# index-tts/index-tts

Measured on AMD Instinct MI355X. Metric: audio-seconds/sec (RTF) IndexTTS-2.5, 64-utt batch @1/2/4/8 MI355X, higher is better.
Workload: dtype bf16 (GPT GEMM operands / KV cache; f32 accumulate, residual stream, norms: the reference's own GPU mode) + fp32x3 (flow matching: f32 activations / weights / accumulation, GEMM and attention products on the bf16 matrix pipe with every f32 operand carried exactly as three bf16 planes = 24 significan

## Files before the change

### indextts_amd/csrc/bigvgan_kernels.hip

```cpp
#include "bigvgan_kernels.h"
#include <stdlib.h>

#define AA_TILE 1024

__global__ __launch_bounds__(256) void aa_act_kernel(const float* __restrict__ x, float* __restrict__ y,
                                                     const float* __restrict__ alpha, const float* __restrict__ beta,
                                                     const float* __restrict__ fu, const float* __restrict__ fd,
                                                     int C, int T, const int* __restrict__ lens, int len_mult,
                                                     int logscale) {
    __shared__ float xs[AA_TILE + 16];
    __shared__ float vs[2 * AA_TILE + 16];
    __shared__ float fus[12], fds[12];
    const int b = blockIdx.z, c = blockIdx.y;
    const int t0 = blockIdx.x * AA_TILE;
    const int len = lens ? min(lens[b] * len_mult, T) : T;
    if (t0 >= len) return;
    const int tid = threadIdx.x;
    if (tid < 12) { fus[tid] = fu[tid]; fds[tid] = fd[tid]; }
    const float* xr = x + ((size_t)b * C + c) * T;
    float* yr = y + ((size_t)b * C + c) * T;
    float a_e = alpha[c], b_e = beta[c];
    if (logscale) { a_e = expf(a_e); b_e = expf(b_e); }
    const float inv_b = 1.0f / (b_e + 1e-9f);
    const int n_out = min(AA_TILE, len - t0);
    for (int i = tid; i < n_out + 12; i += 256) {
        int t = t0 - 6 + i;
        t = t < 0 ? 0 : (t > len - 1 ? len - 1 : t);
        xs[i] = xr[t];
    }
    __syncthreads();
    const int two_len_m1 = 2 * len - 1;
    for (int vi = tid; vi < 2 * n_out + 12; vi += 256) {
        int i = 2 * t0 - 6 + vi;
        i = i < 0 ? 0 : (i > two_len_m1 ? two_len_m1 : i);
        const int q = i >> 1;
        const int base = q - (t0 - 6);
        float u = 0.f;
        if (i & 1) {
#pragma unroll
            for (int j = 0; j < 6; ++j) u = fmaf(fus[2 * j], xs[base + 3 - j], u);
        } else {
#pragma unroll
            for (int j = 0; j < 6; ++j) u = fmaf(fus[1 + 2 * j], xs[base + 2 - j], u);
        }
        u *= 2.0f;
        const float s = sinf(u * a_e);
        vs[vi] = u + inv_b * s * s;
    }
    __syncthreads();
    for (int i = tid; i < n_out; i += 256) {
        float acc = 0.f;
#pragma unroll
        for (int j = 0; j < 12; ++j) acc = fmaf(fds[j], vs[2 * i + j + 1], acc);
        yr[t0 + i] = acc;
    }
}

__device__ __forceinline__ float sin_reduced(float x) {
    const float inv2pi = 0.15915494309189535f;
    const float k = rintf(x * inv2pi);
    float r = fmaf(-k, 6.2831855f, x);
    r = fmaf(-k, -1.7484555e-7f, r);
    return __builtin_amdgcn_sinf(r * inv2pi);
}

__device__ __forceinline__ int aa_sw(int i) { return i ^ (((i >> 6) & 1) << 2); }

template <int OPT, bool FAST_SIN>
__global__ __launch_bounds__(256) void aa_act_kernel_v2(const float* __restrict__ x, float* __restrict__ y,
                                                        const float* __restrict__ alpha, const float* __restrict__ beta,
                                                        const float* __restrict__ fu, const float* __restrict__ fd,
                                                        int C, int T, const int* __restrict__ lens, int len_mult,
                                                        int logscale) {
    constexpr int TILE = 256 * OPT;
    __shared__ __attribute__((aligned(16))) float xs[TILE + 16];
    __shared__ __attribute__((aligned(16))) float vs[2 * TILE + 64];
    const int b = blockIdx.z, c = blockIdx.y;
    const int t0 = blockIdx.x * TILE;
    const int len = lens ? min(lens[b] * len_mult, T) : T;
    if (t0 >= len) return;
    const int tid = threadIdx.x;
    const float* xr = x + ((size_t)b * C + c) * T;
    float* yr = y + ((size_t)b * C + c) * T;
    float fus[12], fds[12];
#pragma unroll
    for (int j = 0; j < 12; ++j) { fus[j] = 2.0f * fu[j]; fds[j] = fd[j]; }
    float a_e = alpha[c], b_e = beta[c];
    if (logscale) { a_e = expf(a_e); b_e = expf(b_e); }
    const float inv_b = 1.0f / (b_e + 1e-9f);
    const int n_out = min(TILE, len - t0);
    float xl[OPT + 1];
#pragma unroll
    for (int k = 0; k < OPT + 1; ++k) {
        int t = t0 - 6 + tid + 256 * k;
        t = t < 0 ? 0 : (t > len - 1 ? len - 1 : t);
        xl[k] = xr[t];
    }
#pragma unroll
    for (int k = 0; k < OPT + 1; ++k)
        if (tid + 256 * k < TILE + 12) xs[tid + 256 * k] = xl[k];
    __syncthreads();
    auto snake8 = [&](int vb, float* v) {
        float xw[12];
        *(f32x4*)&xw[0] = *(const f32x4*)&xs[(vb >> 1)];
        *(f32x4*)&xw[4] = *(const f32x4*)&xs[(vb >> 1) + 4];
        *(f32x4*)&xw[8] = *(const f32x4*)&xs[(vb >> 1) + 8];
#pragma unroll
        for (int p = 0; p < 4; ++p) {
            float ue = 0.f, uo = 0.f;
#pragma unroll
            for (int j = 0; j < 6; ++j) {
                ue = fmaf(fus[1 + 2 * j], xw[p + 5 - j], ue);
                uo = fmaf(fus[2 * j], xw[p + 6 - j], uo);
            }
            const float se = FAST_SIN ? sin_reduced(ue * a_e) : sinf(ue * a_e);
            const float so = FAST_SIN ? sin_reduced(uo * a_e) : sinf(uo * a_e);
            v[2 * p] = fmaf(inv_b * se, se, ue);
            v[2 * p + 1] = fmaf(inv_b * so, so, uo);
        }
    };
#pragma unroll
    for (int g = 0; g < OPT / 4; ++g) {
        float v[8];
        const int vb = 2 * OPT * tid + 8 * g;
        snake8(vb, v);
        *(f32x4*)&vs[aa_sw(vb)] = *(const f32x4*)&v[0];
        *(f32x4*)&vs[aa_sw(vb + 4)] = *(const f32x4*)&v[4];
    }
    if (tid < 2) {
        float vt[8];
        snake8(2 * TILE + 8 * tid, vt);
        *(f32x4*)&vs[aa_sw(2 * TILE + 8 * tid)] = *(const f32x4*)&vt[0];
        *(f32x4*)&vs[aa_sw(2 * TILE + 8 * tid + 4)] = *(const f32x4*)&vt[4];
    }
    __syncthreads();
    if (t0 == 0 && tid < 6) vs[aa_sw(tid)] = vs[aa_sw(6)];
    const int vi_end = (2 * len - 1) - (2 * t0 - 6);
    if (vi_end < 2 * TILE + 12 - 1) {
        const int vi = vi_end + 1 + tid;
        if (tid < 8 && vi < 2 * TILE + 16) vs[aa_sw(vi)] = vs[aa_sw(vi_end)];
    }
    __syncthreads();
#pragma unroll
    for (int g = 0; g < OPT / 4; ++g) {
        float vw[20];
        const int base = 2 * (OPT * tid + 4 * g);
#pragma unroll
        for (int k = 0; k < 5; ++k) *(f32x4*)&vw[4 * k] = *(const f32x4*)&vs[aa_sw(base + 4 * k)];
        f32x4 o;
#pragma unroll
        for (int p = 0; p < 4; ++p) {
            float acc = 0.f;
#pragma unroll
            for (int j = 0; j < 12; ++j) acc = fmaf(fds[j], vw[2 * p + j + 1], acc);
            o[p] = acc;
        }
        const int i0 = OPT * tid + 4 * g;
        if (i0 + 3 < n_out && ((t0 + i0) & 3) == 0 && (T & 3) == 0) {
            *(f32x4*)&yr[t0 + i0] = o;
        } else {
#pragma unroll
            for (int p = 0; p < 4; ++p)
                if (i0 + p < n_out) yr[t0 + i0 + p] = o[p];
        }
    }
}

#define AAP_TT 128
#define AAP_CB 32
#define AAP_RS 36
__device__ __forceinline__ uint32_t aap_cvt2(float a, float b) {
    typedef __bf16 bf2 __attribute__((ext_vector_type(2)));
    typedef float f2 __attribute__((ext_vector_type(2)));
    return __builtin_bit_cast(uint32_t, __builtin_convertvector(f2{a, b}, bf2));
}
__device__ __forceinline__ void aap_wave_sync() {
    __builtin_amdgcn_fence(__ATOMIC_RELEASE, "wavefront");
    __builtin_amdgcn_wave_barrier();
    __builtin_amdgcn_fence(__ATOMIC_ACQUIRE, "wavefront");
}
__device__ __forceinline__ int aap_slot(int tt) { return (tt & 3) * 32 + (tt >> 2); }

__global__ __launch_bounds__(256) void aa_act_planes_kernel(const float* __restrict__ x, u16* __restrict__ xh, u16* __restrict__ xm, u16* __restrict__ xl,
                                                            const float* __restrict__ alpha, const float* __restrict__ beta,
                                                            const float* __restrict__ fu, const float* __restrict__ fd,
                                                            int C, int T, const int* __restrict__ lens, int len_mult, int logscale) {
    __shared__ __attribute__((aligned(256))) float xs[4][2][192];
    __shared__ __attribute__((aligned(256))) float vs[4][2][320];
    __shared__ __attribute__((aligned(16))) u16 ot[3][AAP_TT][AAP_RS];
    const int b = blockIdx.z, c0 = blockIdx.y * AAP_CB, t0 = blockIdx.x * AAP_TT;
    const int tid = threadIdx.x, lane = tid & 63, w = tid >> 6, sub = lane >> 5, pos = lane & 31;
    const int len = lens ? min(lens[b] * len_mult, T) : T;
    const int n_out = len - t0 < AAP_TT ? (len - t0 < 0 ? 0 : len - t0) : AAP_TT;
    if (n_out > 0) {
        float fus[12], fds[12];
#pragma unroll
        for (int j = 0; j < 12; ++j) { fus[j] = 2.0f * fu[j]; fds[j] = fd[j]; }
        float* xw_ = xs[w][sub];
        float* vw_ = vs[w][sub];
        int toff[5];
#pragma unroll
        for (int k = 0; k < 5; ++k) {
            int t = t0 - 6 + pos + 32 * k;
            toff[k] = t < 0 ? 0 : (t > len - 1 ? len - 1 : t);
        }
        auto chan = [&](int it) { const int c = c0 + w * 8 + it * 2 + sub; return c < C ? c : C - 1; };
        float xn[5];
        {
            const float* xr = x + ((size_t)b * C + chan(0)) * T;
#pragma unroll
            for (int k = 0; k < 5; ++k) xn[k] = xr[toff[k]];
        }
#pragma unroll 1
        for (int it = 0; it < 4; ++it) {
            const int cl = w * 8 + it * 2 + sub;
            const bool c_ok = c0 + cl < C;
            float a_e = alpha[chan(it)], b_e = beta[chan(it)];
            if (logscale) { a_e = expf(a_e); b_e = expf(b_e); }
            const float inv_b = 1.0f / (b_e + 1e-9f);
            aap_wave_sync();
#pragma unroll
            for (int k = 0; k < 5; ++k) xw_[pos + 32 * k] = xn[k];
            if (it < 3) {
                const float* xr = x + ((size_t)b * C + chan(it + 1)) * T;
#pragma unroll
                for (int k = 0; k < 5; ++k) xn[k] = xr[toff[k]];
            }
            aap_wave_sync();
            auto snake8 = [&](int vb, float* v) {
                float xw[12];
                *(f32x4*)&xw[0] = *(const f32x4*)&xw_[(vb >> 1)];
                *(f32x4*)&xw[4] = *(const f32x4*)&xw_[(vb >> 1) + 4];
                *(f32x4*)&xw[8] = *(const f32x4*)&xw_[(vb >> 1) + 8];
#pragma unroll
                for (int p = 0; p < 4; ++p) {
                    float ue = 0.f, uo = 0.f;
#pragma unroll
                    for (int j = 0; j < 6; ++j) {
                        ue = fmaf(fus[1 + 2 * j], xw[p + 5 - j], ue);
                        uo = fmaf(fus[2 * j], xw[p + 6 - j], uo);
                    }
                    const float se = sin_reduced(ue * a_e);
                    const float so = sin_reduced(uo * a_e);
                    v[2 * p] = fmaf(inv_b * se, se, ue);
                    v[2 * p + 1] = fmaf(inv_b * so, so, uo);
                }
            };
            {
                float v[8];
                const int vb = 8 * pos;
                snake8(vb, v);
                *(f32x4*)&vw_[aa_sw(vb)] = *(const f32x4*)&v[0];
                *(f32x4*)&vw_[aa_sw(vb + 4)] = *(const f32x4*)&v[4];
            }
            if (pos < 2) {
                float vt[8];
                snake8(2 * AAP_TT + 8 * pos, vt);
                *(f32x4*)&vw_[aa_sw(2 * AAP_TT + 8 * pos)] = *(const f32x4*)&vt[0];
                *(f32x4*)&vw_[aa_sw(2 * AAP_TT + 8 * pos + 4)] = *(const f32x4*)&vt[4];
            }
            aap_wave_sync();
            if (t0 == 0 && pos < 6) vw_[aa_sw(pos)] = vw_[aa_sw(6)];
            const int vi_end = (2 * len - 1) - (2 * t0 - 6);
            if (vi_end < 2 * AAP_TT + 12 - 1) {
                const int vi = vi_end + 1 + pos;
                if (pos < 8 && vi < 2 * AAP_TT + 16) vw_[aa_sw(vi)] = vw_[aa_sw(vi_end)];
            }
            aap_wave_sync();
            float vw[20];
            const int base = 8 * pos;
#pragma unroll
            for (int k = 0; k < 5; ++k) *(f32x4*)&vw[4 * k] = *(const f32x4*)&vw_[aa_sw(base + 4 * k)];
            float o[4];
#pragma unroll
            for (int p = 0; p < 4; ++p) {
                float acc = 0.f;
#pragma unroll
                for (int j = 0; j < 12; ++j) acc = fmaf(fds[j], vw[2 * p + j + 1], acc);
                o[p] = (4 * pos + p < n_out && c_ok) ? acc : 0.f;
            }
#pragma unroll
            for (int e = 0; e < 2; ++e) {
                const float f0 = o[2 * e], f1 = o[2 * e + 1];
                const uint32_t h = aap_cvt2(f0, f1);
                const float r0 = f0 - __uint_as_float(h << 16), r1 = f1 - __uint_as_float(h & 0xffff0000u);
                const uint32_t m = aap_cvt2(r0, r1);
                const float s0 = r0 - __uint_as_float(m << 16), s1 = r1 - __uint_as_float(m & 0xffff0000u);
                const uint32_t l = aap_cvt2(s0, s1);
                const int sa = aap_slot(4 * pos + 2 * e), sb = aap_slot(4 * pos + 2 * e + 1);
                ot[0][sa][cl] = (u16)h; ot[0][sb][cl] = (u16)(h >> 16);
                ot[1][sa][cl] = (u16)m; ot[1][sb][cl] = (u16)(m >> 16);
                ot[2][sa][cl] = (u16)l; ot[2][sb][cl] = (u16)(l >> 16);
            }
        }
    }
    __syncthreads();
    const size_t plane_row = (size_t)b * T;
    const int q = tid & 3;
#pragma unroll 1
    for (int r = tid >> 2; r < 3 * AAP_TT; r += 64) {
        const int p = r / AAP_TT, tt = r - p * AAP_TT;
        const int t = t0 + tt;
        if (t >= T || c0 + 8 * q >= C) continue;
        uint2 lo = {0u, 0u}, hi = {0u, 0u};
        if (n_out > 0) {
            const u16* src = &ot[p][aap_slot(tt)][8 * q];
            lo = *(const uint2*)src;
            hi = *(const uint2*)(src + 4);
        }
        u16* dst = (p == 0 ? xh : (p == 1 ? xm : xl)) + (plane_row + t) * C + c0 + 8 * q;
        *(uint4*)dst = uint4{lo.x, lo.y, hi.x, hi.y};
    }
}

#define CI_CHUNK 32
#define CONV_HALO 64


template <int WM, int WN, int MT, int NT>
__global__ __launch_bounds__(256) __attribute__((amdgpu_waves_per_eu((WM == 1 && MT == 1) ? 4 : 1, (WM == 1 && MT == 1) ? 4 : 8)))
void conv_mfma_kernel(ConvArgs a) {
    constexpr int BM = WM * MT * 32;
    constexpr int BN = WN * NT * 32;
    constexpr int LDW = BN + CONV_HALO;
    extern __shared__ __attribute__((aligned(16))) float xs[];

    const int tid = threadIdx.x, lane = tid & 63, w = tid >> 6;
    const int wm = w / WN, wn = w % WN;
    const int L = blockIdx.x;
    const int xcd = L & 7, slot = L >> 3;
    const int tile = (slot / a.n_co) * 8 + xcd;
    if (tile >= a.n_mt * a.B) return;
    const int b = tile / a.n_mt;
    const int m0 = (tile - b * a.n_mt) * BN;
    const int co0 = (slot % a.n_co) * BM;
    const int len_in = a.lens ? min(a.lens[b] * a.len_mult_in, a.Tin) : a.Tin;
    const int len_out = a.lens ? min(a.lens[b] * a.len_mult_out, a.Tout) : a.Tout;
    const int m_count = len_in + a.m_extra;
    if (m0 >= m_count) return;

    const int span = (a.k - 1) * (a.tap_step < 0 ? -a.tap_step : a.tap_step);
    const int last_off = a.tap_base + (a.k - 1) * a.tap_step;
    const int min_off = a.tap_base < last_off ? a.tap_base : last_off;
    const int W = BN + span;
    const int n_cosub = (a.Cout + 31) >> 5;
    const int cin8 = a.Cin >> 3;

    f32x16 acc[MT][NT];
#pragma unroll
    for (int i = 0; i < MT; ++i)
#pragma unroll
        for (int j = 0; j < NT; ++j)
#pragma unroll
            for (int r = 0; r < 16; ++r) acc[i][j][r] = 0.f;

    const float* xb = a.x + (size_t)b * a.Cin * a.Tin;
    const int lane_row = lane >> 5;
    const int lane_col = lane & 31;

    constexpr int NCOL = LDW / 64;
    float stage[CI_CHUNK / 4][NCOL];
    const int w_u = __builtin_amdgcn_readfirstlane(w);
    auto stage_load = [&](int ci0s) {
        const int cnt = min(CI_CHUNK, a.Cin - ci0s);
#pragma unroll
        for (int rr = 0; rr < CI_CHUNK / 4; ++rr) {
            const int r = w_u + 4 * rr;
            const bool row_ok = r < cnt;
            const float* xr = xb + (size_t)(ci0s + (row_ok ? r : 0)) * a.Tin;
            const __amdgpu_buffer_rsrc_t rsrc =
                __builtin_amdgcn_make_buffer_rsrc(const_cast<float*>(xr), 0, row_ok ? len_in * 4 : 0, 0x00020000);
#pragma unroll
            for (int i = 0; i < NCOL; ++i) {
                const int t = m0 + min_off + lane + 64 * i;
                stage[rr][i] = __builtin_bit_cast(float, __builtin_amdgcn_raw_buffer_load_b32(rsrc, t * 4, 0, 0));
            }
        }
    };
    auto stage_write = [&]() {
#pragma unroll
        for (int rr = 0; rr < CI_CHUNK / 4; ++rr)
#pragma unroll
            for (int i = 0; i < NCOL; ++i) xs[(w + 4 * rr) * LDW + lane + 64 * i] = stage[rr][i];
    };
    stage_load(0);

    constexpr int CP4 = CI_CHUNK / 8;
    f32x4 a_cur[CP4][MT], a_nxt[CP4][MT];
    const int nchunks = (a.Cin + CI_CHUNK - 1) / CI_CHUNK;
    const int G = nchunks * a.k;
    const unsigned wpk_bytes = (unsigned)n_cosub * a.k * cin8 * 64u * 16u;
    const __amdgpu_buffer_rsrc_t wrs = __builtin_amdgcn_make_buffer_rsrc(const_cast<float*>(a.wpk), 0, (int)wpk_bytes, 0x00020000);
    auto load_tap = [&](int g, f32x4 (&dst)[CP4][MT]) {
        const int c = g / a.k, j = g - c * a.k;
        const int cbase = c * CI_CHUNK;
        const int cp4n = min(CI_CHUNK, a.Cin - cbase) >> 3;
#pragma unroll
        for (int cp4 = 0; cp4 < CP4; ++cp4) {
#pragma unroll
            for (int mt = 0; mt < MT; ++mt) {
                const int co_sub = (co0 >> 5) + wm * MT + mt;
                const bool ok = (cp4 < cp4n) && (co_sub < n_cosub);
                const unsigned off = ok ? ((unsigned)((co_sub * a.k + j) * cin8 + ((cbase >> 3) + cp4)) * 64u + lane) * 16u
                                        : 0xFFFFFFF0u;
                dst[cp4][mt] = __builtin_bit_cast(f32x4, __builtin_amdgcn_raw_buffer_load_b128(wrs, off, 0, 0));
            }
        }
    };
    auto compute_tap = [&](int j) {
        const int colb = wn * NT * 32 + lane_col + (a.tap_base + j * a.tap_step - min_off);
        const float* xcol = xs + lane_row * LDW + colb;
        float bcur[4][NT], bnxt[4][NT];
#pragma unroll
        for (int sidx = 0; sidx < 4; ++sidx)
#pragma unroll
            for (int nt = 0; nt < NT; ++nt) bcur[sidx][nt] = xcol[(2 * sidx) * LDW + nt * 32];
#pragma unroll
        for (int cp4 = 0; cp4 < CP4; ++cp4) {
            if (cp4 + 1 < CP4) {
#pragma unroll
                for (int sidx = 0; sidx < 4; ++sidx)
#pragma unroll
                    for (int nt = 0; nt < NT; ++nt) bnxt[sidx][nt] = xcol[((cp4 + 1) * 8 + 2 * sidx) * LDW + nt * 32];
            }
#pragma unroll
            for (int sidx = 0; sidx < 4; ++sidx)
#pragma unroll
                for (int mt = 0; mt < MT; ++mt)
#pragma unroll
                    for (int nt = 0; nt < NT; ++nt)
                        acc[mt][nt] = __builtin_amdgcn_mfma_f32_32x32x2f32(a_cur[cp4][mt][sidx], bcur[sidx][nt], acc[mt][nt], 0, 0, 0);
            if (cp4 + 1 < CP4) {
#pragma unroll
                for (int sidx = 0; sidx < 4; ++sidx)
#pragma unroll
                    for (int nt = 0; nt < NT; ++nt) bcur[sidx][nt] = bnxt[sidx][nt];
            }
        }
#pragma unroll
        for (int cp4 = 0; cp4 < CP4; ++cp4)
#pragma unroll
            for (int mt = 0; mt < MT; ++mt) a_cur[cp4][mt] = a_nxt[cp4][mt];
    };
    load_tap(0, a_cur);
    int g = 0;
    for (int ci0 = 0; ci0 < a.Cin; ci0 += CI_CHUNK) {
        __syncthreads();
        stage_write();
        __syncthreads();
        load_tap(g + 1 < G ? g + 1 : G - 1, a_nxt);
        stage_load(ci0 + CI_CHUNK);
        compute_tap(0);
        ++g;
        for (int j = 1; j < a.k; ++j, ++g) {
            load_tap(g + 1 < G ? g + 1 : G - 1, a_nxt);
            compute_tap(j);
        }
    }

    const int plane_bytes = a.Cout * a.Tout * 4;
    const __amdgpu_buffer_rsrc_t yrs =
        __builtin_amdgcn_make_buffer_rsrc(a.y + (size_t)b * a.Cout * a.Tout, 0, plane_bytes, 0x00020000);
    const float* resb = a.res ? a.res + (size_t)b * a.Cout * a.Tout : a.y;
    const __amdgpu_buffer_rsrc_t rrs = __builtin_amdgcn_make_buffer_rsrc(const_cast<float*>(resb), 0, plane_bytes, 0x00020000);
#pragma unroll
    for (int mt = 0; mt < MT; ++mt) {
#pragma unroll
        for (int hf = 0; hf < 2; ++hf) {
            int corow[8];
            float badd[8];
#pragma unroll
            for (int q = 0; q < 8; ++q) {
                const int r = hf * 8 + q;
                corow[q] = co0 + (wm * MT + mt) * 32 + (r & 3) + 8 * (r >> 2) + 4 * lane_row;
                badd[q] = 0.f;
            }
            if (a.bias) {
#pragma unroll
                for (int q = 0; q < 8; ++q) badd[q] = a.bias[corow[q] < a.Cout ? corow[q] : a.Cout - 1];
            }
            if (a.bias_b) {
                const float* bb = a.bias_b + (size_t)b * a.Cout;
#pragma unroll
                for (int q = 0; q < 8; ++q) badd[q] += bb[corow[q] < a.Cout ? corow[q] : a.Cout - 1];
            }
#pragma unroll
            for (int nt = 0; nt < NT; ++nt) {
                const int m = m0 + (wn * NT + nt) * 32 + lane_col;
                const int n = m * a.ostride + a.ooff;
                const bool n_ok = (m < m_count) && (n >= 0) && (n < len_out);
                unsigned voff[8];
                float v[8];
#pragma unroll
                for (int q = 0; q < 8; ++q) {
                    const bool ok = n_ok && corow[q] < a.Cout;
                    voff[q] = ok ? (unsigned)(corow[q] * a.Tout + n) * 4u : 0xFFFFFFF0u;
                    v[q] = acc[mt][nt][hf * 8 + q] + badd[q];
                }
                if (a.res) {
                    float rv[8];
#pragma unroll
                    for (int q = 0; q < 8; ++q) rv[q] = __builtin_bit_cast(float, __builtin_amdgcn_raw_buffer_load_b32(rrs, voff[q], 0, 0));
#pragma unroll
                    for (int q = 0; q < 8; ++q) v[q] += rv[q];
                }
                if (a.acc_mode != 0) {
                    float yo[8];
#pragma unroll
                    for (int q = 0; q < 8; ++q) yo[q] = __builtin_bit_cast(float, __builtin_amdgcn_raw_buffer_load_b32(yrs, voff[q], 0, 0));
#pragma unroll
                    for (int q = 0; q < 8; ++q) v[q] = a.acc_mode == 1 ? yo[q] + v[q] : (yo[q] + v[q]) / a.div;
                }
#pragma unroll
                for (int q = 0; q < 8; ++q) __builtin_amdgcn_raw_buffer_store_b32(__builtin_bit_cast(unsigned, v[q]), yrs, voff[q], 0, 0);
            }
        }
    }
}

__global__ __launch_bounds__(256) void conv_post_kernel(const float* __restrict__ x, float* __restrict__ y,
                                                        const float* __restrict__ w, const float* __restrict__ bias,
                                                        int Cin, int T, int k, const int* __restrict__ lens,
                                                        int len_mult, int use_tanh) {
    extern __shared__ float ws[];
    const int b = blockIdx.y;
    for (int i = threadIdx.x; i < Cin * k; i += 256) ws[i] = w[i];
    __syncthreads();
    const int t = blockIdx.x * 256 + threadIdx.x;
    if (t >= T) return;
    const int len = lens ? min(lens[b] * len_mult, T) : T;
    float acc = 0.f;
    if (t < len) {
        const int pad = (k - 1) / 2;
        acc = bias ? bias[0] : 0.f;
        const float* xb = x + (size_t)b * Cin * T;
        for (int ci = 0; ci < Cin; ++ci) {
            const float* xr = xb + (size_t)ci * T;
            for (int j = 0; j < k; ++j) {
                const int tt = t + j - pad;
                if (tt >= 0 && tt < len) acc = fmaf(ws[ci * k + j], xr[tt], acc);
            }
        }
        acc = use_tanh ? tanhf(acc) : fminf(1.0f, fmaxf(-1.0f, acc));
    }
    y[(size_t)b * T + t] = acc;
}

__global__ __launch_bounds__(256) void cond_bias_kernel(const float* __restrict__ spk, const float* __restrict__ w,
                                                        const float* __restrict__ bias, float* __restrict__ out,
                                                        int Cout, int cond_dim) {
    const int b = blockIdx.y;
    const int co = blockIdx.x * 256 + threadIdx.x;
    if (co >= Cout) return;
    float acc = bias ? bias[co] : 0.f;
    const float* wr = w + (size_t)co * cond_dim;
    const float* sr = spk + (size_t)b * cond_dim;
    for (int d = 0; d < cond_dim; ++d) acc = fmaf(wr[d], sr[d], acc);
    out[(size_t)b * Cout + co] = acc;
}

int launch_aa_act(const float* x, float* y, const float* alpha, const float* beta, const float* fu, const float* fd,
                  int B, int C, int T, const int* lens, int len_mult, int logscale, hipStream_t st) {
    if (B <= 0 || C <= 0 || T <= 0) return ITTS_OK;
    const int mode = itts_opt(OPT_AA_ACT);
    if (mode == 0) hipLaunchKernelGGL(aa_act_kernel, dim3(ceil_div(T, AA_TILE), C, B), dim3(256), 0, st, x, y, alpha, beta, fu, fd, C, T, lens, len_mult, logscale);
    else if (mode == 1) hipLaunchKernelGGL((aa_act_kernel_v2<4, false>), dim3(ceil_div(T, 1024), C, B), dim3(256), 0, st, x, y, alpha, beta, fu, fd, C, T, lens, len_mult, logscale);
    else if (mode == 2) hipLaunchKernelGGL((aa_act_kernel_v2<4, true>), dim3(ceil_div(T, 1024), C, B), dim3(256), 0, st, x, y, alpha, beta, fu, fd, C, T, lens, len_mult, logscale);
    else hipLaunchKernelGGL((aa_act_kernel_v2<8, true>), dim3(ceil_div(T, 2048), C, B), dim3(256), 0, st, x, y, alpha, beta, fu, fd, C, T, lens, len_mult, logscale);
    HIP_TRY(hipGetLastError());
    return ITTS_OK;
}

int launch_aa_act_planes(const float* x, void* xp, const float* alpha, const float* beta, const float* fu, const float* fd,
                         int B, int C, int T, const int* lens, int len_mult, int logscale, hipStream_t st) {
    if (B <= 0 || C <= 0 || T <= 0) return ITTS_OK;
    if (C % 8) { itts_set_error("aa_act_planes: C %% 8 != 0"); return ITTS_ERR_ARG; }
    u16* p = (u16*)xp;
    const size_t plane = (size_t)B * T * C;
    hipLaunchKernelGGL(aa_act_planes_kernel, dim3(ceil_div(T, AAP_TT), ceil_div(C, AAP_CB), B), dim3(256), 0, st, x, p, p + plane, p + 2 * plane,
                       alpha, beta, fu, fd, C, T, lens, len_mult, logscale);
    HIP_TRY(hipGetLastError());
    return ITTS_OK;
}

template <int WM, int WN, int MT, int NT>
static int launch_conv_cfg(const ConvArgs& a, int B, int m_total, hipStream_t st) {
    constexpr int BM = WM * MT * 32, BN = WN * NT * 32;
    const size_t lds = (size_t)CI_CHUNK * (BN + CONV_HALO) * sizeof(float);
    ConvArgs a2 = a;
    a2.B = B;
    a2.n_mt = ceil_div(m_total, BN);
    a2.n_co = ceil_div(a.Cout, BM);
    const long long tiles8 = ((long long)a2.n_mt * B + 7) / 8 * 8;
    const long long nblocks = tiles8 * a2.n_co;
    if (nblocks > 2147483647ll) { itts_set_error("conv: grid too large"); return ITTS_ERR_ARG; }
    hipLaunchKernelGGL((conv_mfma_kernel<WM, WN, MT, NT>), dim3((unsigned)nblocks), dim3(256), lds, st, a2);
    HIP_TRY(hipGetLastError());
    return ITTS_OK;
}

int launch_conv(const ConvArgs& a, int B, hipStream_t st) {
    if (B <= 0) return ITTS_OK;
    if (a.Cin % 8 != 0) { itts_set_error("conv: C_in=%d must be a multiple of 8", a.Cin); return ITTS_ERR_ARG; }
    if ((long long)a.Cout * a.Tout >= (1ll << 29)) { itts_set_error("conv: C_out*T_out = %lld exceeds the 2 GiB per-row plane limit", (long long)a.Cout * a.Tout); return ITTS_ERR_ARG; }
    if ((long long)a.Tin >= (1ll << 29)) { itts_set_error("conv: T too large"); return ITTS_ERR_ARG; }
    const int span = (a.k - 1) * (a.tap_step < 0 ? -a.tap_step : a.tap_step);
    if (span > CONV_HALO) { itts_set_error("conv: tap span %d exceeds halo %d", span, CONV_HALO); return ITTS_ERR_ARG; }
    const int m_total = a.Tin + a.m_extra;
    const int n_cosub = (a.Cout + 31) / 32;
    const int force_bm = itts_opt(OPT_CONV_BM);
    const int bm_sub = force_bm ? force_bm / 32 : 1;
    (void)n_cosub;
    switch (bm_sub) {
        case 1: return launch_conv_cfg<1, 4, 1, 2>(a, B, m_total, st);
        case 2: return launch_conv_cfg<1, 4, 2, 2>(a, B, m_total, st);
        case 3: return launch_conv_cfg<1, 4, 3, 2>(a, B, m_total, st);
        default: return launch_conv_cfg<2, 2, 2, 2>(a, B, m_total, st);
    }
}

int launch_conv_post(const float* x, float* y, const float* w, const float* bias, int B, int Cin, int T, int k,
                     const int* lens, int len_mult, int use_tanh, hipStream_t st) {
    if (B <= 0 || T <= 0) return ITTS_OK;
    dim3 grid(ceil_div(T, 256), B);
    hipLaunchKernelGGL(conv_post_kernel, grid, dim3(256), (size_t)Cin * k * sizeof(float), st, x, y, w, bias, Cin, T, k,
                       lens, len_mult, use_tanh);
    HIP_TRY(hipGetLastError());
    return ITTS_OK;
}

int launch_cond_bias(const float* spk, const float* w, const float* bias, float* out, int B, int Cout, int cond_dim,
                     hipStream_t st) {
    if (B <= 0 || Cout <= 0) return ITTS_OK;
    dim3 grid(ceil_div(Cout, 256), B);
    hipLaunchKernelGGL(cond_bias_kernel, grid, dim3(256), 0, st, spk, w, bias, out, Cout, cond_dim);
    HIP_TRY(hipGetLastError());
    return ITTS_OK;
}
```

### indextts_amd/csrc/common.h

```cpp
#pragma once
#include <hip/hip_runtime.h>
#include <stdint.h>
#include <stdio.h>
#include <string.h>

#define ITTS_OK 0
#define ITTS_ERR_ARG 1
#define ITTS_ERR_HIP 2
#define ITTS_ERR_STATE 3
#define ITTS_ERR_NOMEM 4

#define HIP_TRY(expr)                                                                         \
    do {                                                                                      \
        hipError_t _e = (expr);                                                               \
        if (_e != hipSuccess) {                                                               \
            itts_set_error("%s:%d %s -> %s", __FILE__, __LINE__, #expr, hipGetErrorString(_e)); \
            return ITTS_ERR_HIP;                                                              \
        }                                                                                     \
    } while (0)

void itts_set_error(const char* fmt, ...);

enum { OPT_DECODE_FUSE_LN, OPT_DECODE_GEMM, OPT_DECODE_ROT, OPT_DECODE_WNT, OPT_DECODE_NT, OPT_PREFILL_GEMM, OPT_TILE256, OPT_F32_TILE,
       OPT_X3_PRODUCTS, OPT_X3_SCHED, OPT_X3_ATTN, OPT_SAMPLE_RADIX, OPT_GPT_COMPACT, OPT_ATTN_WAVES, OPT_S2MEL_FUSED, OPT_FA_QS,
       OPT_F32_ATTN_SCALAR, OPT_FA32_QS, OPT_AA_ACT, OPT_CONV_BM, OPT_H3_KERNEL, OPT_DECODE_LN_NT, OPT_X3_APLANES, OPT_X3_PIN, OPT_PREFILL_ATTN, OPT_VOC_ACT_PLANES, OPT_X3_WAVES, OPT_S2MEL_PRUNE_LAST, OPT_X3_ATTN_SKIP, OPT_COUNT };
int itts_opt(int id);
unsigned itts_opt_epoch();

typedef float f32x4 __attribute__((ext_vector_type(4)));
typedef float f32x16 __attribute__((ext_vector_type(16)));
typedef short bf16x8 __attribute__((ext_vector_type(8)));
typedef unsigned short u16;

static inline int ceil_div(int a, int b) { return (a + b - 1) / b; }

struct ItDevGuard {
    int prev = -1;
    bool switched = false;
    explicit ItDevGuard(int dev) {
        if (dev < 0) return;
        if (hipGetDevice(&prev) != hipSuccess) { prev = -1; (void)hipGetLastError(); }
        if (prev != dev && hipSetDevice(dev) == hipSuccess) switched = true;
    }
    ~ItDevGuard() { if (switched && prev >= 0) (void)hipSetDevice(prev); }
    ItDevGuard(const ItDevGuard&) = delete;
    ItDevGuard& operator=(const ItDevGuard&) = delete;
};
static inline int itts_current_device() {
    int d = -1;
    if (hipGetDevice(&d) != hipSuccess) { d = -1; (void)hipGetLastError(); }
    return d;
}
static inline int itts_ptr_device(const void* p) {
    hipPointerAttribute_t at;
    if (!p || hipPointerGetAttributes(&at, p) != hipSuccess) { (void)hipGetLastError(); return -1; }
    return at.type == hipMemoryTypeDevice ? at.device : -1;
}

template <class T>
struct ItPerDevice {
    T v[32] = {};
    T& cur() {
        const int d = itts_current_device();
        return v[(d >= 0 && d < 32) ? d : 0];
    }
};

#ifdef __HIPCC__
__device__ __forceinline__ float wave_sum(float v) {
#pragma unroll
    for (int o = 32; o > 0; o >>= 1) v += __shfl_xor(v, o, 64);
    return v;
}
__device__ __forceinline__ float wave_max(float v) {
#pragma unroll
    for (int o = 32; o > 0; o >>= 1) v = fmaxf(v, __shfl_xor(v, o, 64));
    return v;
}
__device__ __forceinline__ float bf16_to_f32(u16 h) { return __uint_as_float(((uint32_t)h) << 16); }
__device__ __forceinline__ u16 f32_to_bf16(float f) {
    uint32_t u = __float_as_uint(f);
    if ((u & 0x7fffffffu) > 0x7f800000u) return (u16)((u >> 16) | 0x40);
    u += 0x7fffu + ((u >> 16) & 1u);
    return (u16)(u >> 16);
}
#endif

static inline u16 host_f32_to_bf16(float f) {
    uint32_t u;
    memcpy(&u, &f, 4);
    if ((u & 0x7fffffffu) > 0x7f800000u) return (u16)((u >> 16) | 0x40);
    u += 0x7fffu + ((u >> 16) & 1u);
    return (u16)(u >> 16);
}
```

### indextts_amd/csrc/options.hip

```cpp
#include <atomic>
#include <stdlib.h>
#include <string.h>

#include "../../include/indextts_hip.h"
#include "common.h"

namespace {
struct OptDef {
    const char* name;
    int def, lo, hi;
    const char* doc;
    const char* allowed = nullptr;
};
const OptDef kDefs[OPT_COUNT] = {
    {"decode_fuse_ln", 1, 0, 2, "GPT decode: LayerNorm (+ split-K reduce, bias, residual) inside the consuming GEMM -- 1: steps of 1-8 rows (measured faster), 2: up to 16 rows (measured slower above 8, kept for the A/B record), 0: separate ln_kernel launches; bitwise equal"},
    {"decode_gemm", 1, 0, 1, "bf16 decode GEMMs on the LDS-DMA slab kernel (0: register-path gemm_kernel; bitwise equal)"},
    {"decode_rot", 1, 0, 1, "per-block rotation of the slab DMA issue order in the decode GEMM (same bytes, same LDS image)"},
    {"decode_wnt", 0, 0, 1, "non-temporal policy on the decode GEMM's weight stream"},
    {"decode_nt", 0, 0, 4, "force the n-tiles per block of the 64-row decode GEMM (0: smallest that fits one round of blocks)", "0,1,2,4"},
    {"prefill_gemm", 1, 0, 1, "bf16 prefill GEMMs on the LDS-DMA tile kernels (0: register-path gemm_kernel; bitwise equal)"},
    {"tile256", -1, -1, 2, "bf16 tile GEMM: -1 pick by shape, 0 always 128x128, 1 always 256x256, 2 always 256x128 (bitwise equal)"},
    {"f32_tile", 1, 0, 1, "f32 GEMMs with plain epilogues on the f32-MFMA tile kernel (0: register-path kernel; bitwise equal)"},
    {"x3_products", 6, 6, 8, "plane products per f32 product of the fp32x3 GEMMs and attention: 6 (hh, hm, mh, hl, lh, mm; drops m*l and l*m, 2^-24 |ab| each: measured error vs f64 <= the native f32-MFMA kernels' on every benchmarked shape) or 8 (every term down to 2^-24 |ab|; two blocks per CU like the default since the packed-RoPE fix -- option x3_pin = 1 restores round 4's one-block pin as a diagnostic)", "6,8"},
    {"x3_sched", 1, 0, 1, "fp32x3 GEMM: interleave the operand split with the MFMAs (0: split as a burst; bitwise equal)"},
    {"x3_attn", 1, 0, 1, "fp32x3 s2mel: attention products on bf16 planes too (K / V^T written as three planes by the wqkv epilogue, flash_attn_x3_kernel); 0: the f32-MFMA flash kernel"},
    {"sample_radix", -1, -1, 1, "top-k threshold: -1 per-kernel default (radix select in sample_kernel, ballot bisection in the beam kernels), 0 bisection, 1 radix select (identical ids)"},
    {"gpt_compact", 1, 0, 1, "row compaction of ragged decode batches (0 disables it for every handle; identical ids)"},
    {"attn_waves", 0, 0, 16, "waves per block of the KV-cache attention kernel: 0 pick by shape, else 4 / 8 / 16 (the 16 canonical key streams are mapped onto them; bitwise equal)", "0,4,8,16"},
    {"s2mel_fused", 1, 0, 2, "s2mel: fused GEMM epilogues, sampled when a handle is created -- 1: fused, 0: separate element-wise kernels (2: round 4's spelling of 'the bf16 wqkv epilogue fused too'; the same as 1 since the RoPE fix of round 5)"},
    {"fa_qs", 0, 0, 4, "bf16 flash attention: query sub-tiles per wave (0: pick by shape)", "0,1,2,4"},
    {"f32_attn_scalar", 0, 0, 1, "f32 s2mel attention on the one-wave-per-query reference kernel (the A/B path of the f32 flash kernel)"},
    {"fa32_qs", 2, 1, 2, "f32 flash attention: query sub-tiles per wave"},
    {"aa_act", 2, 0, 2, "anti-aliased activation kernel variant (2: swizzled LDS tiles)"},
    {"conv_bm", 0, 0, 128, "force the co-tile height of conv_mfma_kernel (0: pick by channel count)", "0,32,64,96,128"},
    {"h3_kernel", 1, 0, 1, "f16x3 vocoder conv: 1 window kernel, 0 two-stage kernel"},
    {"decode_ln_nt", 2, 2, 4, "LayerNorm-fused decode GEMM at 5-16 rows (weights on waves 0-3, LayerNorm on waves 4-7): n-tiles per block, 2 or 4 (bitwise equal)", "2,4"},
    {"x3_aplanes", 0, 0, 1, "fp32x3 s2mel: the adaptive-RMSNorm outputs as three bf16 planes in fragment order, wqkv / w1|w3 GEMMs without an operand split (bitwise equal)"},
    {"x3_pin", 0, 0, 1, "fp32x3 GEMM: 1 pins the variants that are not the default one (8 products, burst split) to one block per CU -- round 4's workaround for their run-to-run differences, kept as a diagnostic; not needed since the RoPE fix of round 5 (DESIGN.md section 9)"},
    {"prefill_attn", -1, -1, 1, "attention of S > 1 passes (prefill, latent pass): -1 causal MFMA kernel in the bf16 mode, canonical-stream kernel in the f32 parity mode; 0 canonical-stream kernel (one block per query) always; 1 MFMA kernel in both precisions"},
    {"voc_act_planes", 1, 0, 1, "vocoder, bf16x3 conv mode: the anti-aliased activation in front of an x3 conv writes the conv's three operand planes itself (aa_act_planes_kernel); 0: f32 activation + split pass (bit-identical planes)"},
    {"x3_waves", 8, 4, 8, "fp32x3 GEMM: waves per 128 x 128 block -- 8 (4 x 2, wave tile 32 x 64, weights through LDS: four waves per SIMD at two blocks per CU; 64-utterance solve 314.7 vs 323.0 ms per Euler step, profiles/r06k) or 4 (2 x 2, wave tile 64 x 64, weights in registers: round 5's kernel); bitwise equal", "4,8"},
    {"s2mel_prune_last", 1, 0, 1, "fp32x3 s2mel solve with a tail layout: the LAST DiT layer's attention runs the queries of the tail rows only (keys / values: every frame) and writes the tail layout, its wo / FFN norm / w1|w3 / w2 stages run on the tail rows (residual gathered by a row map in the wo epilogue); the x_in GEMM reads its residual from const_in instead of a copy of it; 0: every row, copy first (bitwise equal)"},
    {"x3_attn_skip", 1, 0, 1, "fp32x3 flash attention: a last key tile with <= 32 valid keys skips the MFMAs of its fully masked half, and a wave whose 32 queries are all out of range only stages its share of K / V^T (0: full tiles, every wave computes; bitwise equal)"},
};
std::atomic<int> g_val[OPT_COUNT];
std::atomic<unsigned> g_epoch{1};
std::atomic<bool> g_init{false};

void ensure_init() {
    if (g_init.load(std::memory_order_acquire)) return;
    static std::atomic_flag once = ATOMIC_FLAG_INIT;
    if (!once.test_and_set()) {
        for (int i = 0; i < OPT_COUNT; ++i) g_val[i].store(kDefs[i].def, std::memory_order_relaxed);
        g_init.store(true, std::memory_order_release);
    } else {
        while (!g_init.load(std::memory_order_acquire)) {}
    }
}
int find(const char* name) {
    if (!name) return -1;
    for (int i = 0; i < OPT_COUNT; ++i)
        if (strcmp(kDefs[i].name, name) == 0) return i;
    return -1;
}
}

int itts_opt(int id) {
    ensure_init();
    return g_val[id].load(std::memory_order_relaxed);
}
unsigned itts_opt_epoch() { return g_epoch.load(std::memory_order_relaxed); }

extern "C" int itts_set_option(const char* name, int value) {
    ensure_init();
    const int i = find(name);
    if (i < 0) { itts_set_error("set_option: unknown option '%s'", name ? name : "(null)"); return ITTS_ERR_ARG; }
    if (value < kDefs[i].lo || value > kDefs[i].hi) {
        itts_set_error("set_option: %s = %d outside [%d, %d]", name, value, kDefs[i].lo, kDefs[i].hi);
        return ITTS_ERR_ARG;
    }
    if (kDefs[i].allowed) {
        bool ok = false;
        for (const char* p = kDefs[i].allowed; *p;) {
            char* end;
            const long v = strtol(p, &end, 10);
            ok |= v == value;
            p = *end == ',' ? end + 1 : end;
        }
        if (!ok) { itts_set_error("set_option: %s = %d is not one of {%s}", name, value, kDefs[i].allowed); return ITTS_ERR_ARG; }
    }
    if (g_val[i].exchange(value) != value) g_epoch.fetch_add(1);
    return ITTS_OK;
}
extern "C" int itts_get_option(const char* name, int* value) {
    ensure_init();
    const int i = find(name);
    if (i < 0 || !value) { itts_set_error("get_option: unknown option '%s'", name ? name : "(null)"); return ITTS_ERR_ARG; }
    *value = g_val[i].load();
    return ITTS_OK;
}
extern "C" int itts_reset_options(void) {
    ensure_init();
    bool changed = false;
    for (int i = 0; i < OPT_COUNT; ++i) changed |= g_val[i].exchange(kDefs[i].def) != kDefs[i].def;
    if (changed) g_epoch.fetch_add(1);
    return ITTS_OK;
}
extern "C" int itts_option_count(void) { return OPT_COUNT; }
extern "C" const char* itts_option_name(int index) { return (index >= 0 && index < OPT_COUNT) ? kDefs[index].name : nullptr; }
extern "C" const char* itts_option_doc(int index) { return (index >= 0 && index < OPT_COUNT) ? kDefs[index].doc : nullptr; }
extern "C" int itts_option_default(int index) { return (index >= 0 && index < OPT_COUNT) ? kDefs[index].def : 0; }
```

Before: 144.0.

## Add narrow-channel f32 MFMA conv kernel for small vocoder resblock convs

```diff
diff --git a/indextts_amd/csrc/bigvgan_kernels.hip b/indextts_amd/csrc/bigvgan_kernels.hip
--- a/indextts_amd/csrc/bigvgan_kernels.hip
+++ b/indextts_amd/csrc/bigvgan_kernels.hip
@@ -518,6 +518,161 @@
     }
 }
 
+#define CN_BN 256
+#define CN_LDW 336
+
+template <int MT, int C8>
+__global__ __launch_bounds__(256) void conv_mfma_narrow_kernel(ConvArgs a) {
+    constexpr int NT = 4;
+    constexpr int RPW = 2 * C8;
+    constexpr int NCOL = (CN_BN + CONV_HALO) / 64;
+    extern __shared__ __attribute__((aligned(16))) float xs[];
+
+    const int tid = threadIdx.x, lane = tid & 63, w = tid >> 6;
+    const int tile = blockIdx.x;
+    const int b = tile / a.n_mt;
+    const int m0 = (tile - b * a.n_mt) * CN_BN;
+    const int len_in = a.lens ? min(a.lens[b] * a.len_mult_in, a.Tin) : a.Tin;
+    const int len_out = a.lens ? min(a.lens[b] * a.len_mult_out, a.Tout) : a.Tout;
+    const int m_count = len_in + a.m_extra;
+    if (m0 >= m_count) return;
+
+    const int last_off = a.tap_base + (a.k - 1) * a.tap_step;
+    const int min_off = a.tap_base < last_off ? a.tap_base : last_off;
+    const int cin8 = a.Cin >> 3;
+    const int n_cosub = (a.Cout + 31) >> 5;
+    const int kk = lane >> 4, col = lane & 15;
+
+    const float* xb = a.x + (size_t)b * a.Cin * a.Tin;
+    const int w_u = __builtin_amdgcn_readfirstlane(w);
+    {
+        float stage[RPW][NCOL];
+#pragma unroll
+        for (int rr = 0; rr < RPW; ++rr) {
+            const int r = w_u + 4 * rr;
+            const bool row_ok = r < a.Cin;
+            const float* xr = xb + (size_t)(row_ok ? r : 0) * a.Tin;
+            const __amdgpu_buffer_rsrc_t rsrc =
+                __builtin_amdgcn_make_buffer_rsrc(const_cast<float*>(xr), 0, row_ok ? len_in * 4 : 0, 0x00020000);
+#pragma unroll
+            for (int i = 0; i < NCOL; ++i) {
+                const int t = m0 + min_off + lane + 64 * i;
+                stage[rr][i] = __builtin_bit_cast(float, __builtin_amdgcn_raw_buffer_load_b32(rsrc, t * 4, 0, 0));
+            }
+        }
+#pragma unroll
+        for (int rr = 0; rr < RPW; ++rr)
+#pragma unroll
+            for (int i = 0; i < NCOL; ++i) xs[(w + 4 * rr) * CN_LDW + lane + 64 * i] = stage[rr][i];
+    }
+
+    f32x4 acc[MT][NT];
+#pragma unroll
+    for (int i = 0; i < MT; ++i)
+#pragma unroll
+        for (int j = 0; j < NT; ++j) acc[i][j] = f32x4{0.f, 0.f, 0.f, 0.f};
+
+    const unsigned wpk_bytes = (unsigned)n_cosub * a.k * cin8 * 64u * 16u;
+    const __amdgpu_buffer_rsrc_t wrs = __builtin_amdgcn_make_buffer_rsrc(const_cast<float*>(a.wpk), 0, (int)wpk_bytes, 0x00020000);
+    f32x4 a_raw[C8][MT];
+    auto load_tap = [&](int j) {
+#pragma unroll
+        for (int c8 = 0; c8 < C8; ++c8)
+#pragma unroll
+            for (int mt = 0; mt < MT; ++mt) {
+                const int cs = mt >> 1;
+                const int pl = 16 * (mt & 1) + col + 32 * (kk & 1);
+                const bool ok = c8 < cin8 && cs < n_cosub;
+                const unsigned off = ok ? ((unsigned)((cs * a.k + j) * cin8 + c8) * 64u + pl) * 16u : 0xFFFFFFF0u;
+                a_raw[c8][mt] = __builtin_bit_cast(f32x4, __builtin_amdgcn_raw_buffer_load_b128(wrs, off, 0, 0));
+            }
+    };
+    load_tap(0);
+    __syncthreads();
+
+    const bool hi = (kk >> 1) != 0;
+    for (int j = 0; j < a.k; ++j) {
+        float a_cur[C8][2][MT];
+#pragma unroll
+        for (int c8 = 0; c8 < C8; ++c8)
+#pragma unroll
+            for (int mt = 0; mt < MT; ++mt) {
+                a_cur[c8][0][mt] = hi ? a_raw[c8][mt][1] : a_raw[c8][mt][0];
+                a_cur[c8][1][mt] = hi ? a_raw[c8][mt][3] : a_raw[c8][mt][2];
+            }
+        load_tap(j + 1 < a.k ? j + 1 : a.k - 1);
+        const float* xcol = xs + kk * CN_LDW + w * (NT * 16) + col + (a.tap_base + j * a.tap_step - min_off);
+#pragma unroll
+        for (int c8 = 0; c8 < C8; ++c8)
+#pragma unroll
+            for (int h = 0; h < 2; ++h) {
+                float bv[NT];
+#pragma unroll
+                for (int nt = 0; nt < NT; ++nt) bv[nt] = xcol[(8 * c8 + 4 * h) * CN_LDW + nt * 16];
+#pragma unroll
+                for (int mt = 0; mt < MT; ++mt)
+#pragma unroll
+                    for (int nt = 0; nt < NT; ++nt)
+                        acc[mt][nt] = __builtin_amdgcn_mfma_f32_16x16x4f32(a_cur[c8][h][mt], bv[nt], acc[mt][nt], 0, 0, 0);
+            }
+    }
+
+    const int plane_bytes = a.Cout * a.Tout * 4;
+    const __amdgpu_buffer_rsrc_t yrs =
+        __builtin_amdgcn_make_buffer_rsrc(a.y + (size_t)b * a.Cout * a.Tout, 0, plane_bytes, 0x00020000);
+    const float* resb = a.res ? a.res + (size_t)b * a.Cout * a.Tout : a.y;
+    const __amdgpu_buffer_rsrc_t rrs = __builtin_amdgcn_make_buffer_rsrc(const_cast<float*>(resb), 0, plane_bytes, 0x00020000);
+#pragma unroll
+    for (int mt = 0; mt < MT; ++mt) {
+        int corow[4];
+        float badd[4];
+#pragma unroll
+        for (int q = 0; q < 4; ++q) {
+            corow[q] = mt * 16 + 4 * kk + q;
+            badd[q] = 0.f;
+        }
+        if (a.bias) {
+#pragma unroll
+            for (int q = 0; q < 4; ++q) badd[q] = a.bias[corow[q] < a.Cout ? corow[q] : a.Cout - 1];
+        }
+        if (a.bias_b) {
+            const float* bb = a.bias_b + (size_t)b * a.Cout;
+#pragma unroll
+            for (int q = 0; q < 4; ++q) badd[q] += bb[corow[q] < a.Cout ? corow[q] : a.Cout - 1];
+        }
+#pragma unroll
+        for (int nt = 0; nt < NT; ++nt) {
+            const int m = m0 + (w * NT + nt) * 16 + col;
+            const int n = m * a.ostride + a.ooff;
+            const bool n_ok = (m < m_count) && (n >= 0) && (n < len_out);
+            unsigned voff[4];
+            float v[4];
+#pragma unroll
+            for (int q = 0; q < 4; ++q) {
+                const bool ok = n_ok && corow[q] < a.Cout;
+                voff[q] = ok ? (unsigned)(corow[q] * a.Tout + n) * 4u : 0xFFFFFFF0u;
+                v[q] = acc[mt][nt][q] + badd[q];
+            }
+            if (a.res) {
+                float rv[4];
+#pragma unroll
+                for (int q = 0; q < 4; ++q) rv[q] = __builtin_bit_cast(float, __builtin_amdgcn_raw_buffer_load_b32(rrs, voff[q], 0, 0));
+#pragma unroll
+                for (int q = 0; q < 4; ++q) v[q] += rv[q];
+            }
+            if (a.acc_mode != 0) {
+                float yo[4];
+#pragma unroll
+                for (int q = 0; q < 4; ++q) yo[q] = __builtin_bit_cast(float, __builtin_amdgcn_raw_buffer_load_b32(yrs, voff[q], 0, 0));
+#pragma unroll
+                for (int q = 0; q < 4; ++q) v[q] = a.acc_mode == 1 ? yo[q] + v[q] : (yo[q] + v[q]) / a.div;
+            }
+#pragma unroll
+            for (int q = 0; q < 4; ++q) __builtin_amdgcn_raw_buffer_store_b32(__builtin_bit_cast(unsigned, v[q]), yrs, voff[q], 0, 0);
+        }
+    }
+}
+
 __global__ __launch_bounds__(256) void conv_post_kernel(const float* __restrict__ x, float* __restrict__ y,
                                                         const float* __restrict__ w, const float* __restrict__ bias,
                                                         int Cin, int T, int k, const int* __restrict__ lens,
@@ -599,6 +754,20 @@
     return ITTS_OK;
 }
 
+template <int MT, int C8>
+static int launch_conv_narrow_cfg(const ConvArgs& a, int B, int m_total, hipStream_t st) {
+    const size_t lds = (size_t)8 * C8 * CN_LDW * sizeof(float);
+    ConvArgs a2 = a;
+    a2.B = B;
+    a2.n_mt = ceil_div(m_total, CN_BN);
+    a2.n_co = 1;
+    const long long nblocks = (long long)a2.n_mt * B;
+    if (nblocks > 2147483647ll) { itts_set_error("conv: grid too large"); return ITTS_ERR_ARG; }
+    hipLaunchKernelGGL((conv_mfma_narrow_kernel<MT, C8>), dim3((unsigned)nblocks), dim3(256), lds, st, a2);
+    HIP_TRY(hipGetLastError());
+    return ITTS_OK;
+}
+
 int launch_conv(const ConvArgs& a, int B, hipStream_t st) {
     if (B <= 0) return ITTS_OK;
     if (a.Cin % 8 != 0) { itts_set_error("conv: C_in=%d must be a multiple of 8", a.Cin); return ITTS_ERR_ARG; }
@@ -611,6 +780,11 @@
     const int force_bm = itts_opt(OPT_CONV_BM);
     const int bm_sub = force_bm ? force_bm / 32 : 1;
     (void)n_cosub;
+    if (itts_opt(OPT_CONV_NARROW) != 0 && !force_bm && a.Cout <= 48 && a.Cin <= 48 && a.ostride == 1 && a.m_extra == 0) {
+        if (a.Cout > 32) return launch_conv_narrow_cfg<3, 6>(a, B, m_total, st);
+        if (a.Cin > 24) return launch_conv_narrow_cfg<2, 6>(a, B, m_total, st);
+        return launch_conv_narrow_cfg<2, 3>(a, B, m_total, st);
+    }
     switch (bm_sub) {
         case 1: return launch_conv_cfg<1, 4, 1, 2>(a, B, m_total, st);
         case 2: return launch_conv_cfg<1, 4, 2, 2>(a, B, m_total, st);
diff --git a/indextts_amd/csrc/common.h b/indextts_amd/csrc/common.h
--- a/indextts_amd/csrc/common.h
+++ b/indextts_amd/csrc/common.h
@@ -23,7 +23,7 @@
 
 enum { OPT_DECODE_FUSE_LN, OPT_DECODE_GEMM, OPT_DECODE_ROT, OPT_DECODE_WNT, OPT_DECODE_NT, OPT_PREFILL_GEMM, OPT_TILE256, OPT_F32_TILE,
        OPT_X3_PRODUCTS, OPT_X3_SCHED, OPT_X3_ATTN, OPT_SAMPLE_RADIX, OPT_GPT_COMPACT, OPT_ATTN_WAVES, OPT_S2MEL_FUSED, OPT_FA_QS,
-       OPT_F32_ATTN_SCALAR, OPT_FA32_QS, OPT_AA_ACT, OPT_CONV_BM, OPT_H3_KERNEL, OPT_DECODE_LN_NT, OPT_X3_APLANES, OPT_X3_PIN, OPT_PREFILL_ATTN, OPT_VOC_ACT_PLANES, OPT_X3_WAVES, OPT_S2MEL_PRUNE_LAST, OPT_X3_ATTN_SKIP, OPT_COUNT };
+       OPT_F32_ATTN_SCALAR, OPT_FA32_QS, OPT_AA_ACT, OPT_CONV_BM, OPT_H3_KERNEL, OPT_DECODE_LN_NT, OPT_X3_APLANES, OPT_X3_PIN, OPT_PREFILL_ATTN, OPT_VOC_ACT_PLANES, OPT_X3_WAVES, OPT_S2MEL_PRUNE_LAST, OPT_X3_ATTN_SKIP, OPT_CONV_NARROW, OPT_COUNT };
 int itts_opt(int id);
 unsigned itts_opt_epoch();
 
diff --git a/indextts_amd/csrc/options.hip b/indextts_amd/csrc/options.hip
--- a/indextts_amd/csrc/options.hip
+++ b/indextts_amd/csrc/options.hip
@@ -42,6 +42,7 @@
     {"x3_waves", 8, 4, 8, "fp32x3 GEMM: waves per 128 x 128 block -- 8 (4 x 2, wave tile 32 x 64, weights through LDS: four waves per SIMD at two blocks per CU; 64-utterance solve 314.7 vs 323.0 ms per Euler step, profiles/r06k) or 4 (2 x 2, wave tile 64 x 64, weights in registers: round 5's kernel); bitwise equal", "4,8"},
     {"s2mel_prune_last", 1, 0, 1, "fp32x3 s2mel solve with a tail layout: the LAST DiT layer's attention runs the queries of the tail rows only (keys / values: every frame) and writes the tail layout, its wo / FFN norm / w1|w3 / w2 stages run on the tail rows (residual gathered by a row map in the wo epilogue); the x_in GEMM reads its residual from const_in instead of a copy of it; 0: every row, copy first (bitwise equal)"},
     {"x3_attn_skip", 1, 0, 1, "fp32x3 flash attention: a last key tile with <= 32 valid keys skips the MFMAs of its fully masked half, and a wave whose 32 queries are all out of range only stages its share of K / V^T (0: full tiles, every wave computes; bitwise equal)"},
+    {"conv_narrow", 1, 0, 1, "vocoder: regular convs with at most 48 channels on both sides (the resblock convs of the 48- and 24-channel stages, every conv mode) on the 16-row f32 MFMA kernel whose M and K extents match the channel count (conv_mfma_narrow_kernel); 0: the 32-row conv_mfma_kernel (same error bound against f64, bits may differ in the summation order)"},
 };
 std::atomic<int> g_val[OPT_COUNT];
 std::atomic<unsigned> g_epoch{1};
```

New measurement: 144.7, median of 6. Within noise of the previous version (+0.5%).
